# refresh-bio/colord

Measured on AMD Instinct MI355X. Metric: input Gbases/s + archive size vs ref, ONT 50 Gb at 1/2/4/8 MI355X, higher is better.
Workload: dtype u64

## Files before the change

colord_amd/csrc/encode_es.hip:

```cpp
#include "objects.hpp"
#include "encode_core.hpp"
#include "align_wave.hpp"
#include "align_rows.hpp"
#include "align_giant.hpp"
#include "emit_wave.hpp"
#include <algorithm>
#include <chrono>
#include <climits>
#include <memory>
#include <vector>

struct cl_anchors;
extern "C" const uint32_t* cl_anchors_n_cands(const cl_anchors* a);
extern "C" const uint32_t* cl_anchors_cands(const cl_anchors* a);
extern "C" const uint64_t* cl_anchors_cand_offsets(const cl_anchors* a);
extern "C" const uint32_t* cl_anchors_data(const cl_anchors* a);

using namespace enc;

namespace {
struct AnchorsV { const uint32_t* n_cands; const uint32_t* cand; const uint64_t* cand_off; const uint32_t* data; };

__global__ void k_read_flags(const uint32_t* __restrict__ n_cands, const uint8_t* __restrict__ has_n, uint32_t n, uint32_t* __restrict__ flag, uint32_t* __restrict__ ncand)
{
	const uint32_t r = blockIdx.x * blockDim.x + threadIdx.x;
	if (r >= n) return;
	const uint32_t nc = has_n[r] ? 0u : n_cands[r];
	flag[r] = nc ? 1u : 0u; ncand[r] = nc;
}
__global__ void k_frames_level0(ArenaV A, AnchorsV AV, uint32_t c, const uint8_t* __restrict__ has_n, uint32_t n, const uint32_t* __restrict__ frame_idx, const uint64_t* __restrict__ cand_base,
                                FrameRec* __restrict__ frames, CandEnt* __restrict__ cands, uint32_t* __restrict__ frame_of_read)
{
	const uint32_t r = blockIdx.x * blockDim.x + threadIdx.x;
	if (r >= n) return;
	const uint32_t nc = has_n[r] ? 0u : AV.n_cands[r];
	if (!nc) { frame_of_read[r] = 0xffffffffu; return; }
	const uint32_t f = frame_idx[r];
	frame_of_read[r] = f;
	FrameRec F; F.read = r; F.level = 0; F.enc_off = 0; F.enc_len = A.lens[r]; F.n_cands = nc; F.first_gap = 0; F.n_gaps = 0; F.pad = 0; F.cand_base = cand_base[r];
	frames[f] = F;
	for (uint32_t j = 0; j < nc; ++j) cands[F.cand_base + j] = cand_level0(AV.cand + ((uint64_t)r * c + j) * 4, AV.cand_off[(uint64_t)r * c + j], AV.data);
}

__global__ void k_frame_gap_counts(const FrameRec* __restrict__ frames, const CandEnt* __restrict__ cands, uint32_t n, uint32_t* __restrict__ counts)
{
	const uint32_t f = blockIdx.x * blockDim.x + threadIdx.x;
	if (f < n) counts[f] = cands[frames[f].cand_base + frames[f].level].n + 1;
}
__global__ void k_frame_first_gaps(FrameRec* __restrict__ frames, const uint32_t* __restrict__ first, uint32_t n, uint32_t n_gaps)
{
	const uint32_t f = blockIdx.x * blockDim.x + threadIdx.x;
	if (f >= n) return;
	frames[f].first_gap = first[f];
	frames[f].n_gaps = (f + 1 < n ? first[f + 1] : n_gaps) - first[f];
}
__global__ void k_gap_geometry(LevelV L, ArenaV R, const uint32_t* __restrict__ data, uint32_t min_part_alt, const uint32_t* __restrict__ first_gap,
                               uint32_t* __restrict__ cap, uint32_t* __restrict__ pend_flag, uint32_t* __restrict__ keys, uint32_t* __restrict__ ids, uint32_t* __restrict__ err)
{
// ... 592 lines not shown
		{
			const uint64_t mine = ok ? pairs : 0;
			const uint64_t p0 = wv::bcast(mine, 0u), p1 = wv::bcast(mine, 16u), p2 = wv::bcast(mine, 32u);
			off = gq == 0 ? 0 : gq == 1 ? p0 : gq == 2 ? p0 + p1 : p0 + p1 + p2;
			if (off + mine > pool_pairs) ok = false;
		}
		if (!ok) { r.n = 0; r.m = 0; }
		ulonglong2* const hist = pool + off;
		lap(5);
		qr::row_stage(r, ok, g, A, R);
		qr::lds_fence();
		lap(0);
		const wv::Sweep sw = qr::row_sweep(r, hist, band);
		__builtin_amdgcn_s_waitcnt(0);
		__builtin_amdgcn_fence(__ATOMIC_SEQ_CST, "workgroup");
		if (ok && (r.shw ? sw.best : sw.score) > band) { ok = false; r.n = 0; r.m = 0; }
		lap(1);
		uint32_t wi, wj, wk;
		qr::row_walk(r, hist, r.shw ? (uint32_t)(sw.end + 1) : r.m, wi, wj, wk, PROF ? &wstat : nullptr);
		qr::lds_fence();
		lap(2);
		const uint32_t pre = wi + wj, K = pre + wk;
		qr::row_convert(r, pre, (uint8_t)(wi ? 1 : 2), wk);
		qr::lds_fence();
		lap(3);
		const uint32_t ref_end = r.shw ? (uint32_t)sw.end : g.kind == GK_FLANK_TINY ? g.use - 1 : 0u;
		uint32_t d_before = 0, seq_off = 0;
		if (r.left && g.kind != GK_INNER)
		{
			const uint32_t ref_offset = (g.nr - 1) - ref_end;
			seq_off = ref_offset - (g.nr - g.use);
			d_before = ref_offset;
		}
		qr::row_refactor_pass(r, K, seq_off, 1);
		qr::row_refactor_pass(r, K, 0, 2);
		lap(4);
		if (ok)
		{
			uint32_t* dst = (uint32_t*)(es_pool + g.es_off); const uint32_t* src = (const uint32_t*)r.es;
			for (uint32_t w = bl; w * 4 < K; w += 16) dst[w] = src[w];
		}
		if (have && bl == 0)
		{
			if (ok) { gaps[gi].es_len = K; gaps[gi].d_before = d_before; }
			else redo[atomicAdd(n_redo, 1u)] = gi;
		}
		qr::lds_fence();
		if (PROF) { const uint32_t smax = qr::max4(r.n ? r.m + nb - 1 : 0); if (lane == 0) { atomicAdd(prof + 9, 1ull); atomicAdd(prof + 10, (unsigned long long)smax); } }
	}
	if (PROF && lane == 0) { atomicAdd(prof + 6, (unsigned long long)wstat.iters); atomicAdd(prof + 7, (unsigned long long)wstat.miss); atomicAdd(prof + 8, (unsigned long long)wstat.hit); }
}


__global__ void k_gap_stats(LevelV L, ArenaV A, EncCfg cfg, const uint32_t* __restrict__ pend_idx, uint32_t* __restrict__ spawn_flag, uint32_t* __restrict__ long_list)
{
	const uint32_t gi = blockIdx.x * blockDim.x + threadIdx.x;
	if (gi >= L.n_gaps) return;
	if (L.gaps[gi].ne >= cfg.min_part_alt) { long_list[gi - pend_idx[gi]] = gi; return; }
	spawn_flag[gi] = gap_finish(L, gi, A, cfg, pend_idx[gi]) ? 1u : 0u;
}
__global__ void k_gap_sums(LevelV L, GapSum* __restrict__ sums, uint32_t* __restrict__ long_ids, unsigned int* __restrict__ n_long)
{
	const uint32_t gi = blockIdx.x * blockDim.x + threadIdx.x;
	if (gi >= L.n_gaps) return;
	const uint32_t k = L.gaps[gi].es_len;
	if (k && k <= SUM_LIMIT) sums[gi] = gap_summary(L.es + L.gaps[gi].es_off, k);
	else if (k) long_ids[atomicAdd(n_long, 1u)] = gi;
}
__global__ __launch_bounds__(256) void k_gap_sums_long(LevelV L, GapSum* __restrict__ sums, const uint32_t* __restrict__ long_ids, const unsigned int* __restrict__ n_long)
{
	const uint32_t n = *n_long, n_waves = gridDim.x * 4;
	for (uint32_t idx = blockIdx.x * 4 + (threadIdx.x >> 6); idx < n; idx += n_waves)
	{
		const uint32_t gi = long_ids[idx];
		const RunEl a = run_of_script_wave(L.es + L.gaps[gi].es_off, L.gaps[gi].es_len);
		if ((threadIdx.x & 63) == 0) sums[gi] = GapSum{ a.hl, a.tl, a.mb, a.mt, a.hs | (a.ts << 8) | (a.single ? 1u << 16 : 0u) };
	}
}
__global__ __launch_bounds__(256) void k_gap_stats_long(LevelV L, ArenaV A, EncCfg cfg, const uint32_t* __restrict__ long_list, uint32_t n_long, uint32_t* __restrict__ spawn_flag)
{
	const uint32_t wi = (blockIdx.x * blockDim.x + threadIdx.x) >> 6, lane = threadIdx.x & 63;
	if (wi >= n_long) return;
	const uint32_t gi = long_list[wi];
	GapRec g = L.gaps[gi];
	char* es = L.es + g.es_off;
	const uint64_t ewb = A.word_off[g.read];
	if (g.kind == GK_TRIVIAL)
	{
		if (g.nr == 0) { for (uint32_t i = lane; i < g.ne; i += 64) es[i] = base_letter(arena_base_at(A, ewb, g.enc_start + i)); g.es_len = g.ne; }
		else g.d_before = g.nr;
		__builtin_amdgcn_s_waitcnt(0);
		__builtin_amdgcn_fence(__ATOMIC_SEQ_CST, "workgroup");
	}
	uint32_t nd = 0;
	for (uint32_t i0 = 0; i0 < g.es_len; i0 += 64)
	{
		const uint32_t i = i0 + lane;
		const uint64_t notd = __ballot(i < g.es_len && es[i] != 'D');
		if (notd) { nd = i0 + (uint32_t)__builtin_ctzll(notd); break; }
		nd = i0 + 64 < g.es_len ? i0 + 64 : g.es_len;
	}
	uint32_t h[9] = { 0, 0, 0, 0, 0, 0, 0, 0, 0 }, hd[4] = { 0, 0, 0, 0 };
	for (uint32_t i = lane * 8; i < g.es_len; i += 512)
	{
		uint64_t w = 0; uint32_t nb = 8;
		if (i + 8 <= g.es_len) __builtin_memcpy(&w, es + i, 8);
		else { nb = g.es_len - i; for (uint32_t y = 0; y < nb; ++y) w |= (uint64_t)(uint8_t)es[i + y] << (8 * y); }
		for (uint32_t y = 0; y < nb; ++y)
		{
			const uint32_t c = es_class((char)((w >> (8 * y)) & 0xffu));
#pragma unroll
			for (int k = 0; k < 9; ++k) h[k] += c == (uint32_t)k;
		}
	}
	if (g.ne)
	{
		const uint32_t s = g.enc_start, last = g.enc_start + g.ne - 1, w0 = s >> 5, w1 = last >> 5;
		for (uint32_t wi2 = w0 + lane; wi2 <= w1; wi2 += 64)
		{
			const uint64_t w = A.packed[ewb + wi2];
			const uint32_t ja = wi2 == w0 ? (s & 31) : 0u, jb = wi2 == w1 ? (last & 31) : 31u;
			const uint64_t from = ja == 0 ? ~0ull : ((1ull << (64 - 2 * ja)) - 1), upto = ~((1ull << (62 - 2 * jb)) - 1);
			const uint64_t v = from & upto & 0x5555555555555555ull, lo = w & 0x5555555555555555ull, hi = (w >> 1) & 0x5555555555555555ull;
			const uint32_t c3 = (uint32_t)__popcll(lo & hi & v), c2 = (uint32_t)__popcll(hi & ~lo & v), c1 = (uint32_t)__popcll(lo & ~hi & v);
			hd[3] += c3; hd[2] += c2; hd[1] += c1; hd[0] += (uint32_t)__popcll(v) - c1 - c2 - c3;
		}
	}
#pragma unroll
	for (int k = 0; k < 9; ++k) for (int o = 32; o; o >>= 1) h[k] += __shfl_xor(h[k], o);
#pragma unroll
	for (int k = 0; k < 4; ++k) for (int o = 32; o; o >>= 1) hd[k] += __shfl_xor(hd[k], o);
	uint32_t n = g.es_len, extra = g.d_before;
	if (nd + g.d_before >= 10) { h[2] -= nd; n -= nd; extra = 0; }
	h[2] += extra;
	double sum_h = 0, sum_d = 0;
#pragma unroll
	for (int i = 0; i < 9; ++i) sum_h += h[i];
#pragma unroll
	for (int i = 0; i < 4; ++i) sum_d += hd[i];
	const double rec_h = 1.0 / sum_h, rec_d = 1.0 / sum_d;
	uint32_t mine = 0;
#pragma unroll
	for (int i = 0; i < 9; ++i) if (lane == (uint32_t)i) mine = h[i];
#pragma unroll
	for (int i = 0; i < 4; ++i) if (lane == 16u + (uint32_t)i) mine = hd[i];
	double term = 0;
	if (mine) { const double p = (double)mine * (lane < 16 ? rec_h : rec_d); term = glibc_log2::log2(p) * p; }
	double e_h = 0, e_d = 0;
#pragma unroll
	for (int i = 0; i < 9; ++i) { const double t = __shfl(term, i, 64); if (h[i]) e_h += t; }
#pragma unroll
	for (int i = 0; i < 4; ++i) { const double t = __shfl(term, 16 + i, 64); if (hd[i]) e_d += t; }
	const bool accept = -e_h * (double)(n + extra) * cfg.cost_mult < -e_d * (double)g.ne;
	g.state = accept ? GS_ES : GS_REJECTED;
	if (lane == 0) { L.gaps[gi] = g; spawn_flag[gi] = accept ? 0u : 1u; }
}
__global__ void k_spawn_mark(LevelV L, const uint32_t* __restrict__ data, EncCfg cfg, uint32_t* __restrict__ flag, uint32_t* __restrict__ ncand)
{
	const uint32_t gi = blockIdx.x * blockDim.x + threadIdx.x;
	if (gi >= L.n_gaps) return;
	ncand[gi] = 0;
	if (!flag[gi]) return;
	const GapRec g = L.gaps[gi];
	const FrameRec F = L.frames[g.frame];
	CandEnt out[16];
	const bool alt = spawn_cands(F, L.cands + F.cand_base, data, g, cfg, out);
	flag[gi] = alt ? 1u : 0u;
	ncand[gi] = alt ? F.n_cands : 0u;
	if (!alt) L.gaps[gi].state = GS_LITERAL;
}
__global__ void k_spawn_fill(LevelV L, const uint32_t* __restrict__ data, EncCfg cfg, const uint32_t* __restrict__ flag_scan, const uint64_t* __restrict__ cand_base,
                             FrameRec* __restrict__ frames_next, CandEnt* __restrict__ cands_next)
{
	const uint32_t gi = blockIdx.x * blockDim.x + threadIdx.x;
	if (gi >= L.n_gaps) return;
	if (cand_base[gi + 1] == cand_base[gi]) return;
	spawn_child(L, gi, data, cfg, flag_scan[gi], cand_base[gi], frames_next, cands_next);
}

__global__ void k_read_base_counts(ArenaV A, const uint8_t* __restrict__ has_n, uint32_t n, uint32_t* __restrict__ counts )
{
	const uint32_t r = (blockIdx.x * blockDim.x + threadIdx.x) >> 6, lane = threadIdx.x & 63;
	if (r >= n) return;
	uint32_t c0 = 0, c1 = 0, c2 = 0, c3 = 0;
	if (!has_n[r])
	{
		const uint32_t len = A.lens[r]; const uint64_t wb = A.word_off[r];
		for (uint32_t w = lane; w * 32 < len; w += 64)
		{
			const uint64_t x = A.packed[wb + w]; const uint32_t cnt = len - w * 32 < 32 ? len - w * 32 : 32;
			const uint64_t lo = x & 0x5555555555555555ull, hi = (x >> 1) & 0x5555555555555555ull;
			const uint64_t valid = cnt == 32 ? 0x5555555555555555ull : (0x5555555555555555ull & ~((1ull << (64 - 2 * cnt)) - 1));
			c0 += __popcll(~hi & ~lo & valid); c1 += __popcll(~hi & lo & valid); c2 += __popcll(hi & ~lo & valid); c3 += __popcll(hi & lo & valid);
		}
	}
	for (int o = 32; o; o >>= 1) { c0 += __shfl_xor(c0, o); c1 += __shfl_xor(c1, o); c2 += __shfl_xor(c2, o); c3 += __shfl_xor(c3, o); }
	if (lane == 0) { counts[4 * r] = c0; counts[4 * r + 1] = c1; counts[4 * r + 2] = c2; counts[4 * r + 3] = c3; }
}
__global__ void k_pend_count(TreeV T, uint32_t n_reads, uint32_t* __restrict__ cnt)
{
	const uint32_t r = blockIdx.x * blockDim.x + threadIdx.x;
	if (r >= n_reads) return;
	const uint32_t f0 = T.frame_of_read[r];
	cnt[r] = f0 == 0xffffffffu ? 0u : pend_walk(T, f0, nullptr);
}
__global__ void k_pend_list(TreeV T, uint32_t n_reads, const uint64_t* __restrict__ off, uint32_t* __restrict__ events)
{
	const uint32_t r = blockIdx.x * blockDim.x + threadIdx.x;
// ... 78 lines not shown
				if (!dec_resc) { dcl0 = __shfl(lg, choose_plain ? 14 : 12); dcl1 = __shfl(lg, choose_plain ? 15 : 13); }
				else
				{
					while (dec_sum > MX) { dec0 = (dec0 + 1) / 2; dec1 = (dec1 + 1) / 2; dec_sum = dec0 + dec1; }
					const double rc = 1.0 / dec_sum;
					dcl0 = dec0 ? -glibc_log2::log2((double)dec0 * rc) : 0.0; dcl1 = dec1 ? -glibc_log2::log2((double)dec1 * rc) : 0.0;
				}
				if (lane == 0) { const uint32_t ev = ev_id[k]; T.lv[ev >> 28].dec[ev & 0x0fffffffu] = choose_plain ? 0 : 1; }
			}
		}
	}
}
__global__ __launch_bounds__(256) void k_emit_count_wave(ArenaV A, TreeV T, uint32_t n_reads, const uint32_t* __restrict__ data, uint32_t* __restrict__ sizes, uint32_t* __restrict__ ntuples)
{
	const uint32_t r = blockIdx.x * 4 + (threadIdx.x >> 6);
	if (r >= n_reads) return;
	if (T.frame_of_read[r] == 0xffffffffu) { if ((threadIdx.x & 63) == 0) { sizes[r] = A.lens[r] + 1; ntuples[r] = A.lens[r] + 1; } return; }
	emit_read_wave<false>(A, T, r, data, sizes, ntuples, nullptr, nullptr);
}
__global__ __launch_bounds__(256) void k_emit_write_wave(ArenaV A, TreeV T, uint32_t n_reads, const uint32_t* __restrict__ data, const uint64_t* __restrict__ es_off, uint8_t* __restrict__ out)
{
	const uint32_t r = blockIdx.x * 4 + (threadIdx.x >> 6);
	if (r >= n_reads || T.frame_of_read[r] == 0xffffffffu) return;
	emit_read_wave<true>(A, T, r, data, nullptr, nullptr, es_off, out);
}
__global__ __launch_bounds__(256) void k_emit_plain(ArenaV A, const uint32_t* __restrict__ inv, const uint8_t* __restrict__ has_n, const uint32_t* __restrict__ frame_of_read, uint32_t n_reads,
                                                   const uint64_t* __restrict__ es_off, uint8_t* __restrict__ out)
{
	const uint32_t r = blockIdx.x * 4 + (threadIdx.x >> 6), lane = threadIdx.x & 63;
	if (r >= n_reads || frame_of_read[r] != 0xffffffffu) return;
	const uint32_t len = A.lens[r]; const uint64_t wb = A.word_off[r];
	uint8_t* o = out + es_off[r];
	if (lane == 0) o[0] = (uint8_t)((has_n[r] ? 11 : 9) << 4);
	for (uint32_t i = lane; i < len; i += 64)
	{
		const uint64_t pw = A.packed[wb + (i >> 5)]; const uint32_t iw = inv[wb + (i >> 5)];
		const bool isn = (iw >> (31 - (i & 31))) & 1u;
		o[1 + i] = (uint8_t)((8u << 4) + (isn ? 4u : (uint32_t)(pw >> (62 - 2 * (i & 31))) & 3u));
	}
}

struct LevelBufs {
	DevBuf<FrameRec> frames; DevBuf<CandEnt> cands; DevBuf<GapRec> gaps; DevBuf<char> es; DevBuf<PendRec> pend; DevBuf<uint8_t> dec; DevBuf<GapSum> sums;
	uint32_t n_frames = 0, n_gaps = 0; uint64_t n_cands = 0;
	LevelV view() { return LevelV{ frames.p, cands.p, gaps.p, es.p, pend.p, dec.p, n_frames, n_gaps, sums.p }; }
};
}
#include "encode_diag.hpp"

namespace {
struct EncKnobs {
	uint32_t small_per_cu, quad_waves;
	uint32_t wave_debug_stage;
	bool no_team_align;
	bool gap_debug, gap_shapes, quad_profile, wave_profile, wave_heartbeat;
	static EncKnobs read()
	{
		auto num = [](const char* name, int dflt, int least) { const char* e = getenv(name); return (uint32_t)(e ? std::max(least, atoi(e)) : dflt); };
		auto on = [](const char* name) { return getenv(name) != nullptr; };
		return EncKnobs{ num("COLORD_HIP_SMALL_PER_CU", 4, 1), num("COLORD_HIP_QUAD_WAVES", 2048, 64), num("COLORD_HIP_WAVE_DEBUG_STAGE", 0, INT_MIN), on("COLORD_HIP_NO_TEAM_ALIGN"),
			on("COLORD_HIP_GAP_DEBUG"), on("COLORD_HIP_GAP_SHAPES"), on("COLORD_HIP_QUAD_PROFILE"), on("COLORD_HIP_WAVE_PROFILE"), on("COLORD_HIP_WAVE_HEARTBEAT") };
	}
};
struct EncCall { cl_ctx* ctx; hipStream_t st; ArenaV A, R; AnchorsV AV; EncCfg cfg; const uint8_t* has_n; uint32_t nr, n_cu; uint32_t* err; EncKnobs knobs; };

struct LevelWork {
	DevBuf<uint32_t> first, capw, pflag, keys, ids; DevBuf<uint64_t> es_off; DevBuf<uint32_t> bounds;
	uint64_t ng = 0, es_total = 0, n_pend = 0;
	LevelV V;
	uint32_t hb[N_CLASSES + 3] = { 0 };
	unsigned long long h_cb[2 * N_CLASSES] = { 0 };
	uint32_t count(uint32_t cls) const { return hb[cls + 1] - hb[cls]; }
	const uint32_t* list(uint32_t cls) const { return ids.p + hb[cls]; }
	double bytes(uint32_t cls) const { return 1.25 * (double)h_cb[cls]; }
	double cells(uint32_t cls) const { return (double)h_cb[N_CLASSES + cls]; }
};
struct SpawnWork { DevBuf<uint32_t> sflag, sncand, long_list, sum_long; DevBuf<uint64_t> cbase; };

struct StreamJoin {
	hipStream_t s = nullptr;
	~StreamJoin() { if (s) (void)hipStreamSynchronize(s); }
	cl_status redo_count(cl_ctx* ctx, const unsigned int* cnt, uint32_t& n_redo)
	{
		unsigned int hc[2];
		HIP_TRY(ctx, hipMemcpyAsync(hc, cnt, 8, hipMemcpyDeviceToHost, s));
		HIP_TRY(ctx, hipStreamSynchronize(s));
		s = nullptr;
		n_redo = hc[1];
		return CL_OK;
	}
};

using Levels = std::vector<std::unique_ptr<LevelBufs>>;
cl_status level0_frames(const EncCall& E, uint32_t* frame_of_read, Levels& levels)
{
	cl_ctx* ctx = E.ctx; const uint32_t nr = E.nr;
	auto L = std::make_unique<LevelBufs>();
	DevBuf<uint32_t> flag, ncand; DEV_ALLOC(ctx, flag, (uint64_t)nr + 1); DEV_ALLOC(ctx, ncand, (uint64_t)nr + 1);
	DevBuf<uint64_t> cbase; DEV_ALLOC(ctx, cbase, (uint64_t)nr + 1);
	LAUNCH(ctx, k_read_flags, grid_for(nr, 256), 256, E.AV.n_cands, E.has_n, nr, flag.p, ncand.p);
	uint64_t nf = 0;
	CL_TRY(dev_exclusive_scan_u64(ctx, ncand.p, cbase.p, nr, &L->n_cands));
	CL_TRY(dev_exclusive_scan_u32(ctx, flag.p, nr, &nf));
	L->n_frames = (uint32_t)nf;
	DEV_ALLOC(ctx, L->frames, nf + 1); DEV_ALLOC(ctx, L->cands, L->n_cands + 1);
	LAUNCH(ctx, k_frames_level0, grid_for(nr, 256), 256, E.A, E.AV, E.cfg.c, E.has_n, nr, (const uint32_t*)flag.p, (const uint64_t*)cbase.p, L->frames.p, L->cands.p, frame_of_read);
	HIP_TRY(ctx, hipGetLastError());
	HIP_TRY(ctx, hipStreamSynchronize(E.st));
	levels.push_back(std::move(L));
	return CL_OK;
}

cl_status level_gaps(const EncCall& E, LevelBufs& L, LevelWork& W)
{
	cl_ctx* ctx = E.ctx;
	DEV_ALLOC(ctx, W.first, (uint64_t)L.n_frames + 1);
	LAUNCH(ctx, k_frame_gap_counts, grid_for(L.n_frames, 256), 256, (const FrameRec*)L.frames.p, (const CandEnt*)L.cands.p, L.n_frames, W.first.p);
	CL_TRY(dev_exclusive_scan_u32(ctx, W.first.p, L.n_frames, &W.ng));
	const uint64_t ng = W.ng;
	if (ng >= (1ull << 32)) return cl_fail(ctx, CL_E_UNSUPPORTED, "cl_encode_reads: more than 2^32 gaps in one call");
	L.n_gaps = (uint32_t)ng;
	LAUNCH(ctx, k_frame_first_gaps, grid_for(L.n_frames, 256), 256, L.frames.p, (const uint32_t*)W.first.p, L.n_frames, L.n_gaps);
	DEV_ALLOC(ctx, L.gaps, ng + 1);
	DEV_ALLOC(ctx, W.capw, ng + 1); DEV_ALLOC(ctx, W.pflag, ng + 1); DEV_ALLOC(ctx, W.keys, ng + 1); DEV_ALLOC(ctx, W.ids, ng + 1);
	LAUNCH(ctx, k_gap_geometry, grid_for(ng, 256), 256, L.view(), E.R, E.AV.data, E.cfg.min_part_alt, (const uint32_t*)W.first.p, W.capw.p, W.pflag.p, W.keys.p, W.ids.p, E.err);
	DEV_ALLOC(ctx, W.es_off, ng + 1);
	CL_TRY(dev_exclusive_scan_u64(ctx, W.capw.p, W.es_off.p, ng, &W.es_total));
	CL_TRY(dev_exclusive_scan_u32(ctx, W.pflag.p, ng, &W.n_pend));
	LAUNCH(ctx, k_gap_offsets, grid_for(ng, 256), 256, L.gaps.p, (const uint64_t*)W.es_off.p, L.n_gaps);
	DEV_ALLOC(ctx, L.es, W.es_total + 16); DEV_ALLOC(ctx, L.pend, W.n_pend + 1); DEV_ALLOC(ctx, L.dec, W.n_pend + 1);
// ... 121 lines not shown
		LAUNCHB(ctx, W.bytes(7), k_giant_stage, n_list, 256, V, W.list(7), (const GapRec*)L.gaps.p, E.A, E.R);
		for (uint32_t ph = 0; ph < phases; ++ph) LAUNCH(ctx, k_giant_level, 1024, 64, V, ph);
		LAUNCH(ctx, k_giant_leaves, leaf_waves, 64, V, scratch.p, per_wave);
		LAUNCH(ctx, k_giant_finish, fin_waves, 64, V, L.gaps.p, L.es.p, scratch.p, fin_per_wave, cnt.p, redo.p, cnt.p + 1);
		HIP_TRY(ctx, hipGetLastError());
		return CL_OK;
	}
	cl_status finish(cl_ctx* ctx, uint32_t& n_redo) { return join.redo_count(ctx, cnt.p, n_redo); }
};

cl_status wave_rounds(const EncCall& E, uint32_t lv, LevelBufs& L, const LevelWork& W, const uint32_t* list, uint32_t n_list, double alg_bytes, double cells, bool level_class)
{
	cl_ctx* ctx = E.ctx; hipStream_t st = E.st;
	if (n_list && E.knobs.gap_debug && level_class) CL_TRY(diag::wave_class_shapes(ctx, st, lv, L, W.hb, list, n_list));
	DevBuf<uint32_t> todo, redo; DEV_ALLOC(ctx, todo, (uint64_t)n_list + 1); DEV_ALLOC(ctx, redo, (uint64_t)n_list + 1);
	DevBuf<unsigned int> cnt; DEV_ALLOC(ctx, cnt, 2);
	uint64_t per_wave = 3ull << 20; uint32_t max_waves = 2048;
	DevBuf<unsigned long long> prof;
	if (E.knobs.wave_profile) { DEV_ALLOC(ctx, prof, 16); HIP_TRY(ctx, hipMemsetAsync(prof.p, 0, 128, st)); }
	uint32_t* hbt_dev = nullptr;
	if (n_list && E.knobs.wave_heartbeat) CL_TRY(diag::wave_heartbeat(ctx, &hbt_dev));
	for (int round = 0; n_list; ++round)
	{
		if (round == 5) return cl_fail(ctx, CL_E_NOMEM, "cl_encode_reads: lane pool exhausted (" + std::to_string(n_list) + " gaps left)");
		const uint32_t waves = std::min<uint32_t>(n_list, max_waves);
		DevBuf<uint8_t> scratch; DEV_ALLOC(ctx, scratch, per_wave * waves);
		HIP_TRY(ctx, hipMemsetAsync(cnt.p, 0, 8, st));
		const auto t_launch = std::chrono::steady_clock::now();
		if (round == 0) ctx->next_cells = cells;
		LAUNCHB(ctx, round == 0 ? alg_bytes : 0.0, k_align_wave, waves, 64, list, n_list, L.gaps.p, L.es.p, E.A, E.R, scratch.p, per_wave, cnt.p, redo.p, cnt.p + 1,
			E.knobs.wave_debug_stage, hbt_dev, prof.p);
		if (prof.p) CL_TRY(diag::wave_profile(ctx, st, prof.p, lv, n_list, waves, t_launch));
		HIP_TRY(ctx, hipGetLastError());
		unsigned int hc[2];
		HIP_TRY(ctx, hipMemcpyAsync(hc, cnt.p, 8, hipMemcpyDeviceToHost, st));
		HIP_TRY(ctx, hipStreamSynchronize(st));
		n_list = hc[1];
		if (n_list)
		{
			HIP_TRY(ctx, hipMemcpyAsync(todo.p, redo.p, (uint64_t)n_list * 4, hipMemcpyDeviceToDevice, st));
			HIP_TRY(ctx, hipStreamSynchronize(st));
			list = todo.p;
			++ctx->gap_paths[10];
		}
		per_wave *= 8; max_waves = std::max<uint32_t>(max_waves / 8, 64);
	}
	return CL_OK;
}

cl_status level_decisions(const EncCall& E, LevelBufs& L, const LevelWork& W, SpawnWork& S)
{
	cl_ctx* ctx = E.ctx; const uint64_t ng = W.ng;
	DEV_ALLOC(ctx, S.sflag, ng + 1); DEV_ALLOC(ctx, S.sncand, ng + 1);
	const uint32_t n_long = (uint32_t)(ng - W.n_pend);
	DEV_ALLOC(ctx, S.long_list, (uint64_t)n_long + 1);
	LAUNCH(ctx, k_gap_stats, grid_for(ng, 64), 64, W.V, E.A, E.cfg, (const uint32_t*)W.pflag.p, S.sflag.p, S.long_list.p);
	if (n_long) LAUNCH(ctx, k_gap_stats_long, grid_for((uint64_t)n_long * 64, 256), 256, W.V, E.A, E.cfg, (const uint32_t*)S.long_list.p, n_long, S.sflag.p);
	DEV_ALLOC(ctx, L.sums, ng + 1);
	DEV_ALLOC(ctx, S.sum_long, ng + 2);
	HIP_TRY(ctx, hipMemsetAsync(S.sum_long.p + ng + 1, 0, 4, E.st));
	LAUNCH(ctx, k_gap_sums, grid_for(ng, 64), 64, W.V, L.sums.p, S.sum_long.p, (unsigned int*)(S.sum_long.p + ng + 1));
	LAUNCH(ctx, k_gap_sums_long, 1024, 256, W.V, L.sums.p, (const uint32_t*)S.sum_long.p, (const unsigned int*)(S.sum_long.p + ng + 1));
	LAUNCH(ctx, k_spawn_mark, grid_for(ng, 64), 64, W.V, E.AV.data, E.cfg, S.sflag.p, S.sncand.p);
	HIP_TRY(ctx, hipGetLastError());
	return CL_OK;
}

cl_status level_spawn(const EncCall& E, const LevelWork& W, SpawnWork& S, Levels& levels)
{
	cl_ctx* ctx = E.ctx; const uint64_t ng = W.ng;
	auto N = std::make_unique<LevelBufs>();
	DEV_ALLOC(ctx, S.cbase, ng + 1);
	uint64_t nf = 0;
	CL_TRY(dev_exclusive_scan_u64(ctx, S.sncand.p, S.cbase.p, ng, &N->n_cands));
	CL_TRY(dev_exclusive_scan_u32(ctx, S.sflag.p, ng, &nf));
	N->n_frames = (uint32_t)nf;
	if (!nf) return CL_OK;
	DEV_ALLOC(ctx, N->frames, nf + 1); DEV_ALLOC(ctx, N->cands, N->n_cands + 1);
	LAUNCH(ctx, k_spawn_fill, grid_for(ng, 64), 64, W.V, E.AV.data, E.cfg, (const uint32_t*)S.sflag.p, (const uint64_t*)S.cbase.p, N->frames.p, N->cands.p);
	HIP_TRY(ctx, hipGetLastError());
	HIP_TRY(ctx, hipStreamSynchronize(E.st));
	levels.push_back(std::move(N));
	return CL_OK;
}

cl_status estimate_and_emit(const EncCall& E, const cl_reads* reads, const Levels& levels, const uint32_t* frame_of_read, const uint32_t* h_pack_bounds, uint32_t n_packs,
                            uint8_t* d_es, uint64_t cap, uint64_t* d_es_off, uint32_t* d_es_ntuples, uint64_t* n_out)
{
	cl_ctx* ctx = E.ctx; const uint32_t nr = E.nr;
	TreeV T; memset(&T, 0, sizeof(T));
	for (size_t i = 0; i < levels.size() && i < 10; ++i) T.lv[i] = levels[i]->view();
	T.frame_of_read = frame_of_read;
	DevBuf<uint32_t> base_counts; DEV_ALLOC(ctx, base_counts, 4ull * nr);
	LAUNCHB(ctx, reads->total_bases / 4.0, k_read_base_counts, grid_for((uint64_t)nr * 64, 256), 256, E.A, E.has_n, nr, base_counts.p);
	DevBuf<uint32_t> d_pb; DEV_ALLOC(ctx, d_pb, (uint64_t)n_packs + 1);
	HIP_TRY(ctx, hipMemcpyAsync(d_pb.p, h_pack_bounds, ((uint64_t)n_packs + 1) * 4, hipMemcpyHostToDevice, E.st));
	DevBuf<uint32_t> ev_cnt; DEV_ALLOC(ctx, ev_cnt, (uint64_t)nr + 1);
	DevBuf<uint64_t> ev_off; DEV_ALLOC(ctx, ev_off, (uint64_t)nr + 1);
	LAUNCH(ctx, k_pend_count, grid_for(nr, 64), 64, T, nr, ev_cnt.p);
	uint64_t n_events = 0;
	CL_TRY(dev_exclusive_scan_u64(ctx, ev_cnt.p, ev_off.p, nr, &n_events));
	DevBuf<uint32_t> events; DEV_ALLOC(ctx, events, n_events + 1);
	LAUNCH(ctx, k_pend_list, grid_for(nr, 64), 64, T, nr, (const uint64_t*)ev_off.p, events.p);
	if (n_packs) LAUNCH(ctx, k_estimator, n_packs, 64, T, (const uint32_t*)d_pb.p, n_packs, (const uint32_t*)reads->lens.p, E.has_n, (const uint32_t*)base_counts.p, (const uint64_t*)ev_off.p, (const uint32_t*)events.p);
	DevBuf<uint32_t> sizes; DEV_ALLOC(ctx, sizes, nr);
	uint64_t total = 0;
	LAUNCHB(ctx, reads->total_bases * 1.25, k_emit_count_wave, grid_for(nr, 4), 256, E.A, T, nr, E.AV.data, sizes.p, d_es_ntuples);
	HIP_TRY(ctx, hipGetLastError());
	CL_TRY(dev_exclusive_scan_u64(ctx, sizes.p, d_es_off, nr, &total));
	*n_out = total;
	if (total > cap || (total && !d_es)) return cl_fail(ctx, CL_E_CAPACITY, "cl_encode_reads: need " + std::to_string(total) + " bytes");
	LAUNCHB(ctx, reads->total_bases * 1.25 + (double)total, k_emit_write_wave, grid_for(nr, 4), 256, E.A, T, nr, E.AV.data, (const uint64_t*)d_es_off, d_es);
	LAUNCH(ctx, k_emit_plain, grid_for(nr, 4), 256, E.A, (const uint32_t*)reads->inv.p, E.has_n, frame_of_read, nr, (const uint64_t*)d_es_off, d_es);
	HIP_TRY(ctx, hipGetLastError());
	HIP_TRY(ctx, hipStreamSynchronize(E.st));
// ... 86 lines not shown
```

Measured before the change: 3.074.

## Fuse gap stats and gap summaries into one 16-lane-group tail kernel

Replaces the per-thread gap stats kernel and per-thread gap summary kernel with one kernel that processes each gap with a 16-lane group. It computes the histogram, run summary, pending record and accept decision in a single pass over each gap's script, reading it 8 bytes per lane. Gaps longer than a row limit are sent to the existing wave-wide kernels through an overflow list. This is meant to remove a second read of the script bytes and the serial per-thread loops, and to improve lane utilisation. In exchange it adds ballot and shuffle run-tracking logic, and it relies on the gap id order held in W.ids.

```diff
diff --git a/colord_amd/csrc/encode_es.hip b/colord_amd/csrc/encode_es.hip
--- a/colord_amd/csrc/encode_es.hip
+++ b/colord_amd/csrc/encode_es.hip
@@ -4,6 +4,7 @@
 #include "align_rows.hpp"
 #include "align_giant.hpp"
 #include "emit_wave.hpp"
+#include "gap_tail.hpp"
 #include <algorithm>
 #include <chrono>
 #include <climits>
@@ -702,20 +703,26 @@
 }
 
 
-__global__ void k_gap_stats(LevelV L, ArenaV A, EncCfg cfg, const uint32_t* __restrict__ pend_idx, uint32_t* __restrict__ spawn_flag, uint32_t* __restrict__ long_list)
-{
-	const uint32_t gi = blockIdx.x * blockDim.x + threadIdx.x;
-	if (gi >= L.n_gaps) return;
-	if (L.gaps[gi].ne >= cfg.min_part_alt) { long_list[gi - pend_idx[gi]] = gi; return; }
-	spawn_flag[gi] = gap_finish(L, gi, A, cfg, pend_idx[gi]) ? 1u : 0u;
-}
-__global__ void k_gap_sums(LevelV L, GapSum* __restrict__ sums, uint32_t* __restrict__ long_ids, unsigned int* __restrict__ n_long)
-{
-	const uint32_t gi = blockIdx.x * blockDim.x + threadIdx.x;
-	if (gi >= L.n_gaps) return;
-	const uint32_t k = L.gaps[gi].es_len;
-	if (k && k <= SUM_LIMIT) sums[gi] = gap_summary(L.es + L.gaps[gi].es_off, k);
-	else if (k) long_ids[atomicAdd(n_long, 1u)] = gi;
+__global__ __launch_bounds__(256) void k_gap_tail(LevelV L, ArenaV A, EncCfg cfg, const uint32_t* __restrict__ ids, const uint32_t* __restrict__ pend_idx, GapSum* __restrict__ sums,
+                                                  uint32_t* __restrict__ spawn_flag, uint32_t row_limit, uint32_t* __restrict__ over_ids, unsigned int* __restrict__ n_over)
+{
+	const uint64_t ri = ((uint64_t)blockIdx.x * 256 + threadIdx.x) >> 4;
+	if (ri >= L.n_gaps) return;
+	const uint32_t gi = ids[ri];
+	const GapRec g = L.gaps[gi];
+	const uint32_t k = g.kind == GK_TRIVIAL && g.nr == 0 ? g.ne : g.es_len;
+	if (k > row_limit) { if ((threadIdx.x & 15) == 0) over_ids[atomicAdd(n_over, 1u)] = gi; return; }
+	gap_tail_group<16, true>(L, A, cfg, gi, g, pend_idx[gi], sums, spawn_flag);
+}
+__global__ __launch_bounds__(256) void k_gap_stats_long(LevelV L, ArenaV A, EncCfg cfg, const uint32_t* __restrict__ pend_idx, const uint32_t* __restrict__ over_ids,
+                                                        const unsigned int* __restrict__ n_over, uint32_t* __restrict__ spawn_flag)
+{
+	const uint32_t n = *n_over, n_waves = gridDim.x * 4;
+	for (uint32_t idx = blockIdx.x * 4 + (threadIdx.x >> 6); idx < n; idx += n_waves)
+	{
+		const uint32_t gi = over_ids[idx];
+		gap_tail_group<64, false>(L, A, cfg, gi, L.gaps[gi], pend_idx[gi], nullptr, spawn_flag);
+	}
 }
 __global__ __launch_bounds__(256) void k_gap_sums_long(LevelV L, GapSum* __restrict__ sums, const uint32_t* __restrict__ long_ids, const unsigned int* __restrict__ n_long)
 {
@@ -726,84 +733,6 @@
 		const RunEl a = run_of_script_wave(L.es + L.gaps[gi].es_off, L.gaps[gi].es_len);
 		if ((threadIdx.x & 63) == 0) sums[gi] = GapSum{ a.hl, a.tl, a.mb, a.mt, a.hs | (a.ts << 8) | (a.single ? 1u << 16 : 0u) };
 	}
-}
-__global__ __launch_bounds__(256) void k_gap_stats_long(LevelV L, ArenaV A, EncCfg cfg, const uint32_t* __restrict__ long_list, uint32_t n_long, uint32_t* __restrict__ spawn_flag)
-{
-	const uint32_t wi = (blockIdx.x * blockDim.x + threadIdx.x) >> 6, lane = threadIdx.x & 63;
-	if (wi >= n_long) return;
-	const uint32_t gi = long_list[wi];
-	GapRec g = L.gaps[gi];
-	char* es = L.es + g.es_off;
-	const uint64_t ewb = A.word_off[g.read];
-	if (g.kind == GK_TRIVIAL)
-	{
-		if (g.nr == 0) { for (uint32_t i = lane; i < g.ne; i += 64) es[i] = base_letter(arena_base_at(A, ewb, g.enc_start + i)); g.es_len = g.ne; }
-		else g.d_before = g.nr;
-		__builtin_amdgcn_s_waitcnt(0);
-		__builtin_amdgcn_fence(__ATOMIC_SEQ_CST, "workgroup");
-	}
-	uint32_t nd = 0;
-	for (uint32_t i0 = 0; i0 < g.es_len; i0 += 64)
-	{
-		const uint32_t i = i0 + lane;
-		const uint64_t notd = __ballot(i < g.es_len && es[i] != 'D');
-		if (notd) { nd = i0 + (uint32_t)__builtin_ctzll(notd); break; }
-		nd = i0 + 64 < g.es_len ? i0 + 64 : g.es_len;
-	}
-	uint32_t h[9] = { 0, 0, 0, 0, 0, 0, 0, 0, 0 }, hd[4] = { 0, 0, 0, 0 };
-	for (uint32_t i = lane * 8; i < g.es_len; i += 512)
-	{
-		uint64_t w = 0; uint32_t nb = 8;
-		if (i + 8 <= g.es_len) __builtin_memcpy(&w, es + i, 8);
-		else { nb = g.es_len - i; for (uint32_t y = 0; y < nb; ++y) w |= (uint64_t)(uint8_t)es[i + y] << (8 * y); }
-		for (uint32_t y = 0; y < nb; ++y)
-		{
-			const uint32_t c = es_class((char)((w >> (8 * y)) & 0xffu));
-#pragma unroll
-			for (int k = 0; k < 9; ++k) h[k] += c == (uint32_t)k;
-		}
-	}
-	if (g.ne)
-	{
-		const uint32_t s = g.enc_start, last = g.enc_start + g.ne - 1, w0 = s >> 5, w1 = last >> 5;
-		for (uint32_t wi2 = w0 + lane; wi2 <= w1; wi2 += 64)
-		{
-			const uint64_t w = A.packed[ewb + wi2];
-			const uint32_t ja = wi2 == w0 ? (s & 31) : 0u, jb = wi2 == w1 ? (last & 31) : 31u;
-			const uint64_t from = ja == 0 ? ~0ull : ((1ull << (64 - 2 * ja)) - 1), upto = ~((1ull << (62 - 2 * jb)) - 1);
-			const uint64_t v = from & upto & 0x5555555555555555ull, lo = w & 0x5555555555555555ull, hi = (w >> 1) & 0x5555555555555555ull;
-			const uint32_t c3 = (uint32_t)__popcll(lo & hi & v), c2 = (uint32_t)__popcll(hi & ~lo & v), c1 = (uint32_t)__popcll(lo & ~hi & v);
-			hd[3] += c3; hd[2] += c2; hd[1] += c1; hd[0] += (uint32_t)__popcll(v) - c1 - c2 - c3;
-		}
-	}
-#pragma unroll
-	for (int k = 0; k < 9; ++k) for (int o = 32; o; o >>= 1) h[k] += __shfl_xor(h[k], o);
-#pragma unroll
-	for (int k = 0; k < 4; ++k) for (int o = 32; o; o >>= 1) hd[k] += __shfl_xor(hd[k], o);
-	uint32_t n = g.es_len, extra = g.d_before;
-	if (nd + g.d_before >= 10) { h[2] -= nd; n -= nd; extra = 0; }
-	h[2] += extra;
-	double sum_h = 0, sum_d = 0;
-#pragma unroll
-	for (int i = 0; i < 9; ++i) sum_h += h[i];
-#pragma unroll
-	for (int i = 0; i < 4; ++i) sum_d += hd[i];
-	const double rec_h = 1.0 / sum_h, rec_d = 1.0 / sum_d;
-	uint32_t mine = 0;
-#pragma unroll
-	for (int i = 0; i < 9; ++i) if (lane == (uint32_t)i) mine = h[i];
-#pragma unroll
-	for (int i = 0; i < 4; ++i) if (lane == 16u + (uint32_t)i) mine = hd[i];
-	double term = 0;
-	if (mine) { const double p = (double)mine * (lane < 16 ? rec_h : rec_d); term = glibc_log2::log2(p) * p; }
-	double e_h = 0, e_d = 0;
-#pragma unroll
-	for (int i = 0; i < 9; ++i) { const double t = __shfl(term, i, 64); if (h[i]) e_h += t; }
-#pragma unroll
-	for (int i = 0; i < 4; ++i) { const double t = __shfl(term, 16 + i, 64); if (hd[i]) e_d += t; }
-	const bool accept = -e_h * (double)(n + extra) * cfg.cost_mult < -e_d * (double)g.ne;
-	g.state = accept ? GS_ES : GS_REJECTED;
-	if (lane == 0) { L.gaps[gi] = g; spawn_flag[gi] = accept ? 0u : 1u; }
 }
 __global__ void k_spawn_mark(LevelV L, const uint32_t* __restrict__ data, EncCfg cfg, uint32_t* __restrict__ flag, uint32_t* __restrict__ ncand)
 {
@@ -988,13 +917,15 @@
 struct EncKnobs {
 	uint32_t small_per_cu, quad_waves;
 	uint32_t wave_debug_stage;
+	uint32_t tail_row_limit;
 	bool no_team_align;
 	bool gap_debug, gap_shapes, quad_profile, wave_profile, wave_heartbeat;
 	static EncKnobs read()
 	{
 		auto num = [](const char* name, int dflt, int least) { const char* e = getenv(name); return (uint32_t)(e ? std::max(least, atoi(e)) : dflt); };
 		auto on = [](const char* name) { return getenv(name) != nullptr; };
-		return EncKnobs{ num("COLORD_HIP_SMALL_PER_CU", 4, 1), num("COLORD_HIP_QUAD_WAVES", 2048, 64), num("COLORD_HIP_WAVE_DEBUG_STAGE", 0, INT_MIN), on("COLORD_HIP_NO_TEAM_ALIGN"),
+		return EncKnobs{ num("COLORD_HIP_SMALL_PER_CU", 4, 1), num("COLORD_HIP_QUAD_WAVES", 2048, 64), num("COLORD_HIP_WAVE_DEBUG_STAGE", 0, INT_MIN),
+			num("COLORD_HIP_TAIL_ROW_LIMIT", (int)SUM_LIMIT, 0), on("COLORD_HIP_NO_TEAM_ALIGN"),
 			on("COLORD_HIP_GAP_DEBUG"), on("COLORD_HIP_GAP_SHAPES"), on("COLORD_HIP_QUAD_PROFILE"), on("COLORD_HIP_WAVE_PROFILE"), on("COLORD_HIP_WAVE_HEARTBEAT") };
 	}
 };
@@ -1011,7 +942,7 @@
 	double bytes(uint32_t cls) const { return 1.25 * (double)h_cb[cls]; }
 	double cells(uint32_t cls) const { return (double)h_cb[N_CLASSES + cls]; }
 };
-struct SpawnWork { DevBuf<uint32_t> sflag, sncand, long_list, sum_long; DevBuf<uint64_t> cbase; };
+struct SpawnWork { DevBuf<uint32_t> sflag, sncand, over_list; DevBuf<uint64_t> cbase; };
 
 struct StreamJoin {
 	hipStream_t s = nullptr;
@@ -1239,15 +1170,15 @@
 {
 	cl_ctx* ctx = E.ctx; const uint64_t ng = W.ng;
 	DEV_ALLOC(ctx, S.sflag, ng + 1); DEV_ALLOC(ctx, S.sncand, ng + 1);
-	const uint32_t n_long = (uint32_t)(ng - W.n_pend);
-	DEV_ALLOC(ctx, S.long_list, (uint64_t)n_long + 1);
-	LAUNCH(ctx, k_gap_stats, grid_for(ng, 64), 64, W.V, E.A, E.cfg, (const uint32_t*)W.pflag.p, S.sflag.p, S.long_list.p);
-	if (n_long) LAUNCH(ctx, k_gap_stats_long, grid_for((uint64_t)n_long * 64, 256), 256, W.V, E.A, E.cfg, (const uint32_t*)S.long_list.p, n_long, S.sflag.p);
 	DEV_ALLOC(ctx, L.sums, ng + 1);
-	DEV_ALLOC(ctx, S.sum_long, ng + 2);
-	HIP_TRY(ctx, hipMemsetAsync(S.sum_long.p + ng + 1, 0, 4, E.st));
-	LAUNCH(ctx, k_gap_sums, grid_for(ng, 64), 64, W.V, L.sums.p, S.sum_long.p, (unsigned int*)(S.sum_long.p + ng + 1));
-	LAUNCH(ctx, k_gap_sums_long, 1024, 256, W.V, L.sums.p, (const uint32_t*)S.sum_long.p, (const unsigned int*)(S.sum_long.p + ng + 1));
+	DEV_ALLOC(ctx, S.over_list, ng + 2);
+	unsigned int* n_over = (unsigned int*)(S.over_list.p + ng + 1);
+	HIP_TRY(ctx, hipMemsetAsync(n_over, 0, 4, E.st));
+	const double tail_bytes = 0.625 * (double)W.es_total + (double)ng * (2 * sizeof(GapRec) + sizeof(GapSum) + 12) + (double)W.n_pend * sizeof(PendRec);
+	LAUNCHB(ctx, tail_bytes, k_gap_tail, grid_for(ng * 16, 256), 256, W.V, E.A, E.cfg, (const uint32_t*)W.ids.p, (const uint32_t*)W.pflag.p, L.sums.p, S.sflag.p,
+		E.knobs.tail_row_limit, S.over_list.p, n_over);
+	LAUNCH(ctx, k_gap_stats_long, 1024, 256, W.V, E.A, E.cfg, (const uint32_t*)W.pflag.p, (const uint32_t*)S.over_list.p, (const unsigned int*)n_over, S.sflag.p);
+	LAUNCH(ctx, k_gap_sums_long, 1024, 256, W.V, L.sums.p, (const uint32_t*)S.over_list.p, (const unsigned int*)n_over);
 	LAUNCH(ctx, k_spawn_mark, grid_for(ng, 64), 64, W.V, E.AV.data, E.cfg, S.sflag.p, S.sncand.p);
 	HIP_TRY(ctx, hipGetLastError());
 	return CL_OK;
diff --git a/colord_amd/csrc/gap_tail.hpp b/colord_amd/csrc/gap_tail.hpp
--- /dev/null
+++ b/colord_amd/csrc/gap_tail.hpp
@@ -0,0 +1,186 @@
+#pragma once
+#include "emit_wave.hpp"
+
+namespace enc {
+
+__device__ inline RunEl run_of_word(uint64_t w, uint32_t nb)
+{
+	const uint32_t f = (uint32_t)w & 0xffu, l = (uint32_t)(w >> (8 * (nb - 1))) & 0xffu;
+	const uint64_t xf = w ^ (0x0101010101010101ull * f);
+	uint32_t hl = xf ? (uint32_t)__builtin_ctzll(xf) >> 3 : 8u;
+	if (hl >= nb) return run_single(f, nb);
+	const uint64_t xl = (w << (8 * (8 - nb))) ^ (0x0101010101010101ull * l);
+	const uint32_t tl = (uint32_t)__builtin_clzll(xl) >> 3;
+	return RunEl{ f, hl, l, tl, nb - hl - tl, nb - hl - tl, 0 };
+}
+template<int W> __device__ inline uint32_t group_sum(uint32_t v)
+{
+#pragma unroll
+	for (int o = W / 2; o; o >>= 1) v += (uint32_t)__shfl_xor((int)v, o);
+	return v;
+}
+
+__device__ inline uint32_t tail_close_run(uint32_t sym, uint32_t len, uint32_t (&dm)[4])
+{
+	if (sym == (uint32_t)'D') { if (len >= 10) { ++dm[2]; return bitlen32(len) + 1; } dm[0] += len; }
+	else if (sym == (uint32_t)'M') { if (len >= 15) { ++dm[3]; return bitlen32(len) + 1; } dm[1] += len; }
+	return 0;
+}
+
+__device__ inline void tail_store_gap(GapRec& dst, const GapRec& g, uint32_t state, uint32_t aux)
+{
+	dst.d_before = g.d_before; dst.es_len = g.es_len; dst.state = state; dst.aux = aux;
+}
+
+template<int W, bool SUMS>
+__device__ inline void gap_tail_group(const LevelV& L, const ArenaV& A, const EncCfg& cfg, uint32_t gi, GapRec g, uint32_t pend_slot,
+                                      GapSum* __restrict__ sums, uint32_t* __restrict__ spawn_flag)
+{
+	const uint32_t gl = threadIdx.x & (W - 1), group_at = (threadIdx.x & 63u) & ~(uint32_t)(W - 1);
+	char* es = L.es + g.es_off;
+	const uint64_t ewb = A.word_off[g.read];
+	const bool letters = g.kind == GK_TRIVIAL && g.nr == 0;
+	if (g.kind == GK_TRIVIAL) { if (g.nr == 0) g.es_len = g.ne; else g.d_before = g.nr; }
+	const bool pending = g.ne < cfg.min_part_alt;
+	const uint32_t k = g.es_len;
+	uint32_t h[9] = { 0, 0, 0, 0, 0, 0, 0, 0, 0 }, hd[4] = { 0, 0, 0, 0 }, dm[4] = { 0, 0, 0, 0 };
+	uint32_t first_len = 0, mid_b = 0, mid_t = 0, head_sym = 0;
+	uint32_t carry_sym = 0, carry_len = 0;
+	uint64_t lens = 0;
+	for (uint32_t x0 = 0; x0 < k; x0 += 8 * W)
+	{
+		const uint32_t x = x0 + gl * 8;
+		uint64_t w = 0; uint32_t nb = 0;
+		if (x < k)
+		{
+			nb = k - x < 8 ? k - x : 8;
+			if (letters)
+			{
+				for (uint32_t y = 0; y < nb; ++y) w |= (uint64_t)(uint8_t)base_letter(arena_base_at(A, ewb, g.enc_start + x + y)) << (8 * y);
+				if (nb == 8) __builtin_memcpy(es + x, &w, 8);
+				else for (uint32_t y = 0; y < nb; ++y) es[x + y] = (char)((w >> (8 * y)) & 0xffu);
+			}
+			else if (nb == 8) __builtin_memcpy(&w, es + x, 8);
+			else for (uint32_t y = 0; y < nb; ++y) w |= (uint64_t)(uint8_t)es[x + y] << (8 * y);
+		}
+		const RunEl e = nb ? run_of_word(w, nb) : run_empty();
+		if (x0 == 0) head_sym = (uint32_t)__shfl((int)e.hs, 0, W);
+		uint32_t osym = (uint32_t)__shfl_up((int)e.ts, 1, W);
+		if (gl == 0) osym = carry_sym;
+		const bool starts = nb && !(e.single && e.hs == osym);
+		const uint64_t below = ((__ballot(starts) >> group_at) & (W == 64 ? ~0ull : (1ull << (W & 63)) - 1)) & ((1ull << gl) - 1);
+		const uint32_t at = below ? 63u - (uint32_t)__builtin_clzll(below) : 0u;
+		const uint32_t tl_at = (uint32_t)__shfl((int)e.tl, (int)at, W);
+		uint32_t olen = below ? tl_at + 8 * (gl - 1 - at) : carry_len + 8 * gl, long_term = 0;
+		if (pending && x == 0 && g.d_before && e.hs != (uint32_t)'D') long_term = tail_close_run((uint32_t)'D', g.d_before, dm);
+		const uint64_t code4 = ((w ^ (w >> 4)) & 0x0f0f0f0f0f0f0f0full) << 2;
+		uint64_t cnt = 0;
+#pragma unroll
+		for (int j = 0; j < 8; ++j)
+		{
+			if (j >= (int)nb) break;
+			const uint32_t c = (uint32_t)(w >> (8 * j)) & 0xffu;
+			const bool nw = c != osym;
+			if (nw)
+			{
+				if (olen)
+				{
+					const bool first = x + j == olen;
+					if (first) first_len = olen; else { mid_b += run_bytes((char)osym, olen); mid_t += run_tuples((char)osym, olen); }
+					if (pending)
+					{
+						const uint32_t t = tail_close_run(osym, olen + (first && osym == (uint32_t)'D' ? g.d_before : 0u), dm);
+						if (t) long_term = t;
+					}
+				}
+				osym = c; olen = 0;
+			}
+			++olen;
+			if (!pending || nw) cnt += 1ull << ((uint32_t)(code4 >> (8 * j)) & 63u);
+		}
+		h[0] += (uint32_t)(cnt >> 20) & 15u; h[1] += (uint32_t)(cnt >> 28) & 15u; h[2] += (uint32_t)cnt & 15u; h[3] += (uint32_t)(cnt >> 12) & 15u;
+		h[4] += (uint32_t)(cnt >> 36) & 15u; h[5] += (uint32_t)(cnt >> 4) & 15u; h[6] += (uint32_t)(cnt >> 52) & 15u; h[7] += (uint32_t)(cnt >> 48) & 15u;
+		h[8] += (uint32_t)(cnt >> 60) & 15u;
+		const uint32_t last_lane = (k - x0 - 1) >> 3 < (uint32_t)(W - 1) ? (k - x0 - 1) >> 3 : (uint32_t)(W - 1);
+		carry_sym = (uint32_t)__shfl((int)osym, (int)last_lane, W); carry_len = (uint32_t)__shfl((int)olen, (int)last_lane, W);
+		if (pending)
+		{
+			uint64_t m = (__ballot(long_term != 0) >> group_at) & (W == 64 ? ~0ull : (1ull << (W & 63)) - 1);
+			while (m) { lens_push(lens, (uint32_t)__shfl((int)long_term, (int)__builtin_ctzll(m), W)); m &= m - 1; }
+		}
+	}
+	if (g.ne)
+	{
+		const uint32_t s = g.enc_start, last = g.enc_start + g.ne - 1, w0 = s >> 5, w1 = last >> 5;
+		for (uint32_t wi = w0 + gl; wi <= w1; wi += W)
+		{
+			const uint64_t w = A.packed[ewb + wi];
+			const uint32_t ja = wi == w0 ? (s & 31) : 0u, jb = wi == w1 ? (last & 31) : 31u;
+			const uint64_t from = ja == 0 ? ~0ull : ((1ull << (64 - 2 * ja)) - 1), upto = ~((1ull << (62 - 2 * jb)) - 1);
+			const uint64_t v = from & upto & 0x5555555555555555ull, lo = w & 0x5555555555555555ull, hi = (w >> 1) & 0x5555555555555555ull;
+			const uint32_t c3 = (uint32_t)__popcll(lo & hi & v), c2 = (uint32_t)__popcll(hi & ~lo & v), c1 = (uint32_t)__popcll(lo & ~hi & v);
+			hd[3] += c3; hd[2] += c2; hd[1] += c1; hd[0] += (uint32_t)__popcll(v) - c1 - c2 - c3;
+		}
+	}
+#pragma unroll
+	for (int q = 0; q < 9; ++q) h[q] = group_sum<W>(h[q]);
+#pragma unroll
+	for (int q = 0; q < 4; ++q) hd[q] = group_sum<W>(hd[q]);
+	const bool one_run = k && carry_len == k;
+	if (!one_run) { first_len = group_sum<W>(first_len); mid_b = group_sum<W>(mid_b); mid_t = group_sum<W>(mid_t); }
+	else { first_len = k; mid_b = mid_t = 0; }
+	if (SUMS && k && gl == 0) sums[gi] = GapSum{ first_len, carry_len, mid_b, mid_t, head_sym | (carry_sym << 8) | (one_run ? 1u << 16 : 0u) };
+	if (pending)
+	{
+#pragma unroll
+		for (int q = 0; q < 4; ++q) dm[q] = group_sum<W>(dm[q]);
+		uint32_t t = 0;
+		if (k) t = tail_close_run(carry_sym, carry_len + (one_run && carry_sym == (uint32_t)'D' ? g.d_before : 0u), dm);
+		else if (g.d_before) t = tail_close_run((uint32_t)'D', g.d_before, dm);
+		if (t) lens_push(lens, t);
+		if (gl == 0)
+		{
+			PendRec p;
+			p.rd[0] = h[0]; p.rd[1] = h[1]; p.rd[2] = h[3]; p.rd[3] = h[5]; p.rd[4] = dm[0]; p.rd[5] = dm[1];
+			p.rd[6] = h[6]; p.rd[7] = h[7]; p.rd[8] = h[8]; p.rd[9] = dm[2]; p.rd[10] = dm[3]; p.rd[11] = 0;
+			p.pl[0] = hd[0]; p.pl[1] = hd[1]; p.pl[2] = hd[2]; p.pl[3] = hd[3];
+			p.ref_len = g.nr; p.pad = 0; p.lens = lens;
+			L.pend[pend_slot] = p;
+			tail_store_gap(L.gaps[gi], g, GS_PENDING, pend_slot); spawn_flag[gi] = 0u;
+		}
+		return;
+	}
+	const uint32_t nd = k && head_sym == (uint32_t)'D' ? first_len : 0u;
+	uint32_t n = g.es_len, extra = g.d_before;
+	if (nd + g.d_before >= 10) { h[2] -= nd; n -= nd; extra = 0; }
+	h[2] += extra;
+	double sum_h = 0, sum_d = 0;
+#pragma unroll
+	for (int i = 0; i < 9; ++i) sum_h += h[i];
+#pragma unroll
+	for (int i = 0; i < 4; ++i) sum_d += hd[i];
+	const double rec_h = 1.0 / sum_h, rec_d = 1.0 / sum_d;
+	constexpr int ROUNDS = (13 + W - 1) / W;
+	double term[ROUNDS];
+#pragma unroll
+	for (int r = 0; r < ROUNDS; ++r)
+	{
+		const uint32_t idx = gl + (uint32_t)(r * W);
+		uint32_t mine = 0;
+#pragma unroll
+		for (int i = 0; i < 9; ++i) if (idx == (uint32_t)i) mine = h[i];
+#pragma unroll
+		for (int i = 0; i < 4; ++i) if (idx == 9u + (uint32_t)i) mine = hd[i];
+		term[r] = 0;
+		if (mine) { const double p = (double)mine * (idx < 9 ? rec_h : rec_d); term[r] = glibc_log2::log2(p) * p; }
+	}
+	double e_h = 0, e_d = 0;
+#pragma unroll
+	for (int i = 0; i < 9; ++i) { const double t = __shfl(term[i / W], i % W, W); if (h[i]) e_h += t; }
+#pragma unroll
+	for (int i = 0; i < 4; ++i) { const double t = __shfl(term[(9 + i) / W], (9 + i) % W, W); if (hd[i]) e_d += t; }
+	const bool accept = -e_h * (double)(n + extra) * cfg.cost_mult < -e_d * (double)g.ne;
+	if (gl == 0) { tail_store_gap(L.gaps[gi], g, accept ? GS_ES : GS_REJECTED, g.aux); spawn_flag[gi] = accept ? 0u : 1u; }
+}
+
+}
```

Result: faster. 3.160 (median of 6 runs) (+2.8%).
